# pjookim/srsran-ce-pytorch

Measured on AMD Instinct MI355X. Metric: slots/sec (273-PRB PUSCH, 4 Rx), higher is better.
Workload: dtype f32; 1 GPU; pusch273_4rx_filter; n_prb=273, n_sc=3276, n_sym=14, layers=1, rx_ports=4, smoothing=filter, interp=linear, slots_per_gpu=8192, global_slots=8192, rx_layout=[slot][port][sym][sc], parallelism=slot-shard x1, no collective

## Files before the change

srsran_ce_pytorch_amd/csrc/ce_denoise.hip:

```cpp
#include <hip/hip_runtime.h>
#include <stdint.h>
#include <string.h>

#include <type_traits>
#include <vector>

#include "ce_denoise.h"
#include "ce_stage.h"

typedef _Float16 half8 __attribute__((ext_vector_type(8)));
typedef _Float16 half4 __attribute__((ext_vector_type(4)));
typedef _Float16 half2v __attribute__((ext_vector_type(2)));
typedef float f32x4 __attribute__((ext_vector_type(4)));

struct ce_denoiser {
  int device = 0;
  half8* wfrag = nullptr;
  float* bias = nullptr;
};

#ifndef DN_ABLATE
#define DN_ABLATE 0
#endif

namespace {

#ifndef DN_MIN_WAVES
#define DN_MIN_WAVES 3
#endif
#ifndef DN_TWO_BODIES
#define DN_TWO_BODIES 0
#endif
#ifndef DN_L3_BUF
#define DN_L3_BUF 2
#endif
#ifndef DN_T_ROWS
#define DN_T_ROWS 32
#endif
constexpr int DN_T = DN_T_ROWS;
constexpr int DN_NB3 = DN_T / 16;
static_assert(DN_T % 16 == 0, "strip height");
constexpr int DN_NT = 256, DN_COLS = 16, DN_C = CE_DN_CHANNELS;
constexpr int X0_PIX = (DN_T + 6) * DN_COLS + 2;
constexpr int X1_PIX = (DN_T + 5) * DN_COLS + 2;
constexpr int X2_PIX = (DN_T + 2) * DN_COLS + 2;

__device__ __forceinline__ int tap_off(int tap) {
  const int ky = tap / 3, kx = tap - 3 * ky;
  return (ky - 1) * DN_COLS + (kx - 1);
}

constexpr int ROW_BYTES16 = DN_COLS * DN_C * 2;
constexpr int ROW_BYTES0 = DN_COLS * 4;

typedef _Float16 half2x __attribute__((ext_vector_type(2)));
__device__ __forceinline__ float2 masked(float2 v, bool ok) {
  const unsigned m = ok ? 0xFFFFFFFFu : 0u;
  return make_float2(__uint_as_float(__float_as_uint(v.x) & m), __uint_as_float(__float_as_uint(v.y) & m));
}
__device__ __forceinline__ half4 relu_h4(f32x4 acc, unsigned keep) {
  half2x lo = half2x{(_Float16)acc[0], (_Float16)acc[1]}, hi = half2x{(_Float16)acc[2], (_Float16)acc[3]};
  const half2x z = half2x{0, 0}, top = half2x{65504, 65504};
  lo = __builtin_elementwise_min(__builtin_elementwise_max(lo, z), top);
  hi = __builtin_elementwise_min(__builtin_elementwise_max(hi, z), top);
  unsigned ulo, uhi;
  __builtin_memcpy(&ulo, &lo, 4);
  __builtin_memcpy(&uhi, &hi, 4);
  ulo &= keep;
  uhi &= keep;
  __builtin_memcpy(&lo, &ulo, 4);
  __builtin_memcpy(&hi, &uhi, 4);
  return half4{lo[0], lo[1], hi[0], hi[1]};
}

__global__ __launch_bounds__(DN_NT, DN_MIN_WAVES) void ce_denoise_kernel(float2* __restrict__ ch, const half8* __restrict__ wfrag,
                                                            const float* __restrict__ bias, int n_sc, int L) {
  __shared__ __attribute__((aligned(16))) half2v x0[2][X0_PIX];
  __shared__ __attribute__((aligned(16))) _Float16 x1[X1_PIX * DN_C];
  __shared__ __attribute__((aligned(16))) _Float16 x2[X2_PIX * DN_C];
  const int tid = threadIdx.x, lane = tid & 63;
  const int wave = __builtin_amdgcn_readfirstlane(tid >> 6);
  const int n = lane & 15, g = lane >> 4;
  const int64_t plane = blockIdx.x;
  const int64_t item = plane / L;
  const int l = (int)(plane - item * L);
  float2* base = ch + item * (int64_t)n_sc * CE_DN_SYMBOLS * L + l;

  half8 w1 = wfrag[lane], w2[5], w3[9];
#pragma unroll
  for (int m = 0; m < 5; ++m) w2[m] = wfrag[(1 + m) * 64 + lane];
#pragma unroll
  for (int m = 0; m < 9; ++m) w3[m] = wfrag[(6 + m) * 64 + lane];
  f32x4 b1, b2, b3;
#pragma unroll
  for (int i = 0; i < 4; ++i) {
    b1[i] = bias[4 * g + i];
    b2[i] = bias[16 + 4 * g + i];
    b3[i] = g < 2 ? bias[32 + (i & 1)] : 0.f;
  }
  for (int i = tid; i < 2 * X0_PIX; i += DN_NT) (&x0[0][0])[i] = half2v{0, 0};
  for (int i = tid; i < X1_PIX * DN_C; i += DN_NT) x1[i] = 0;
  for (int i = tid; i < X2_PIX * DN_C; i += DN_NT) x2[i] = 0;

  const bool col_ok = n >= 1 && n <= CE_DN_SYMBOLS;
  const unsigned keep = col_ok ? 0xFFFFFFFFu : 0u;
  int rd0[4];
#pragma unroll
  for (int q = 0; q < 4; ++q) {
    const int tap = 4 * g + q;
    rd0[q] = (1 + (wave + 1) * DN_COLS + n + tap_off(tap < 9 ? tap : 4)) * 4;
  }
  constexpr int R2 = (DN_T + 2 + 3) / 4;
  const int a2 = wave * R2 < DN_T + 2 - R2 ? wave * R2 : DN_T + 2 - R2;
  int rdA, rdC, wr2;
  {
    const int pa = 1 + a2 * DN_COLS + n - 1 + (g >> 1), pc = 1 + (a2 + (g >> 1)) * DN_COLS + n + 1, pw = 1 + a2 * DN_COLS + n;
    rdA = pa * (DN_C * 2) + (((g & 1) ^ ((pa >> 2) & 1)) * 16);
    rdC = pc * (DN_C * 2) + (((g & 1) ^ ((pc >> 2) & 1)) * 16);
    wr2 = pw * (DN_C * 2) + ((((g >> 1) & 1) ^ ((pw >> 2) & 1)) * 16) + (g & 1) * 8;
  }
  const int wpix = 1 + wave * DN_COLS + n;
  const int wr = wpix * (DN_C * 2) + ((((g >> 1) & 1) ^ ((wpix >> 2) & 1)) * 16) + (g & 1) * 8;
  constexpr int ST_N = ((DN_T + 6) * DN_COLS + DN_NT - 1) / DN_NT;
  int st_off[ST_N], st_row[ST_N];
  bool st_ok[ST_N];
#pragma unroll
  for (int k = 0; k < ST_N; ++k) {
    const int i = tid + k * DN_NT, sym = (i & 15) - 1;
    st_row[k] = (i >> 4) - 3;
    st_ok[k] = i < (DN_T + 6) * DN_COLS && sym >= 0 && sym < CE_DN_SYMBOLS;
    st_off[k] = (st_row[k] * CE_DN_SYMBOLS + sym) * L;
  }
  int rd3[3];
#pragma unroll
  for (int dx = 0; dx < 3; ++dx) {
    const int pix = 1 + (4 * wave + 3 * (g >> 1)) * DN_COLS + n + dx - 1;
    rd3[dx] = pix * (DN_C * 2) + (((g & 1) ^ ((pix >> 2) & 1)) * 16);
  }
  const int h_row = 4 * wave + 2 * g;
  const int h_off = (h_row * CE_DN_SYMBOLS + (n - 1)) * L;
  const bool h_lane = g < 2 && col_ok;

  float2 st[ST_N];
  auto stage_load = [&](int r0) {
    const float2* sb = base + (int64_t)r0 * CE_DN_SYMBOLS * L;
#pragma unroll
    for (int k = 0; k < ST_N; ++k) {
      const bool ok = st_ok[k] && (unsigned)(r0 + st_row[k]) < (unsigned)n_sc;
      st[k] = masked((DN_ABLATE & 2) ? make_float2(0.f, 0.f) : sb[ok ? st_off[k] : 0], ok);
    }
  };
  auto stage_load_in = [&](int r0) {
    const float2* sb = base + (int64_t)r0 * CE_DN_SYMBOLS * L;
#pragma unroll
    for (int k = 0; k < ST_N; ++k) st[k] = masked((DN_ABLATE & 2) ? make_float2(0.f, 0.f) : sb[st_ok[k] ? st_off[k] : 0], st_ok[k]);
  };
  auto stage_store = [&](int buf) {
#pragma unroll
    for (int k = 0; k < ST_N; ++k) {
      const int i = tid + k * DN_NT;
      if (i < (DN_T + 6) * DN_COLS) x0[buf][1 + i] = half2v{(_Float16)st[k].x, (_Float16)st[k].y};
    }
  };
  stage_load(0);
  __syncthreads();
  stage_store(0);
  __syncthreads();
  const int n_strips = (n_sc + DN_T - 1) / DN_T;
  auto strip = [&](auto edge_tag, int s) __attribute__((always_inline)) {
    constexpr bool EDGE = decltype(edge_tag)::value;
    const int r0 = s * DN_T, buf = s & 1;
    float2* sb = base + (int64_t)r0 * CE_DN_SYMBOLS * L;
    if (s + 1 < n_strips) {
      if (!EDGE && r0 + 2 * DN_T + 3 <= n_sc) stage_load_in(r0 + DN_T); else stage_load(r0 + DN_T);
    }
    float2 hres[DN_NB3][2];
#pragma unroll
    for (int b = 0; b < DN_NB3; ++b)
#pragma unroll
      for (int e = 0; e < 2; ++e) {
        const bool ok = h_lane && (!EDGE || r0 + h_row + 16 * b + e < n_sc);
        hres[b][e] = masked((DN_ABLATE & 2) ? make_float2(0.f, 0.f) : sb[ok ? h_off + (16 * b + e) * CE_DN_SYMBOLS * L : 0], ok);
      }
    {
      const char* xin = reinterpret_cast<const char*>(&x0[buf][0]);
      char* xout = reinterpret_cast<char*>(x1);
      constexpr int NK1 = (DN_T + 4) / 4;
      auto finish1 = [&](f32x4 acc, int k) __attribute__((always_inline)) {
        const int row = r0 - 2 + wave + 4 * k;
        const unsigned rowkeep = (!EDGE || (row >= 0 && row < n_sc)) ? keep : 0u;
        *reinterpret_cast<half4*>(xout + wr + k * 4 * ROW_BYTES16) = relu_h4(acc, rowkeep);
      };
      f32x4 accp = b1;
      half2v px[2][4];
#pragma unroll
      for (int q = 0; q < 4; ++q) px[0][q] = *reinterpret_cast<const half2v*>(xin + rd0[q]);
#pragma unroll
      for (int k = 0; k < NK1; ++k) {
        if (k + 1 < NK1) {
#pragma unroll
          for (int q = 0; q < 4; ++q) px[(k + 1) & 1][q] = *reinterpret_cast<const half2v*>(xin + rd0[q] + (k + 1) * 4 * ROW_BYTES0);
        }
        asm volatile("" ::: "memory");
        half8 b;
#pragma unroll
        for (int q = 0; q < 4; ++q) {
          b[2 * q] = px[k & 1][q][0];
          b[2 * q + 1] = px[k & 1][q][1];
        }
        const f32x4 acc = __builtin_amdgcn_mfma_f32_16x16x32_f16(w1, b, b1, 0, 0, 0);
        if (k > 0) finish1(accp, k - 1);
        accp = acc;
      }
      finish1(accp, NK1 - 1);
    }
    __syncthreads();
    if (s + 1 < n_strips) stage_store(buf ^ 1);
    {
      const char* xin = reinterpret_cast<const char*>(x1);
      char* xout = reinterpret_cast<char*>(x2);
      half8 fa[R2 + 2], fc[R2 + 2];
      auto fetch = [&](int i) __attribute__((always_inline)) {
        fa[i] = *reinterpret_cast<const half8*>(xin + rdA + i * ROW_BYTES16);
        fc[i] = *reinterpret_cast<const half8*>(xin + rdC + i * ROW_BYTES16);
      };
      fetch(0);
      fetch(1);
      fetch(2);
      auto finish2 = [&](f32x4 acc, int j) __attribute__((always_inline)) {
        const int row = r0 - 1 + a2 + j;
        const unsigned rowkeep = (!EDGE || (row >= 0 && row < n_sc)) ? keep : 0u;
        *reinterpret_cast<half4*>(xout + wr2 + j * ROW_BYTES16) = relu_h4(acc, rowkeep);
      };
      f32x4 accp = b2;
#pragma unroll
      for (int j = 0; j < R2; ++j) {
        if (j + 3 < R2 + 2) fetch(j + 3);
        asm volatile("" ::: "memory");
        f32x4 acc = b2;
        acc = __builtin_amdgcn_mfma_f32_16x16x32_f16(w2[0], fa[j], acc, 0, 0, 0);
        acc = __builtin_amdgcn_mfma_f32_16x16x32_f16(w2[1], fa[j + 1], acc, 0, 0, 0);
        acc = __builtin_amdgcn_mfma_f32_16x16x32_f16(w2[2], fa[j + 2], acc, 0, 0, 0);
        acc = __builtin_amdgcn_mfma_f32_16x16x32_f16(w2[3], fc[j], acc, 0, 0, 0);
        acc = __builtin_amdgcn_mfma_f32_16x16x32_f16(w2[4], fc[j + 2], acc, 0, 0, 0);
        if (j > 0) finish2(accp, j - 1);
        accp = acc;
      }
      finish2(accp, R2 - 1);
    }
    __syncthreads();
    {
      const char* xin = reinterpret_cast<const char*>(x2);
      auto finish3 = [&](f32x4 acc, int b) __attribute__((always_inline)) {
#pragma unroll
        for (int e = 0; e < 2; ++e)
          if ((!(DN_ABLATE & 1) || acc[0] == 123.456f) && h_lane && (!EDGE || r0 + h_row + 16 * b + e < n_sc))
            sb[h_off + (16 * b + e) * CE_DN_SYMBOLS * L] = make_float2(hres[b][e].x + acc[2 * e], hres[b][e].y + acc[2 * e + 1]);
      };
      f32x4 accp = b3;
      half8 fr[DN_L3_BUF][9];
#pragma unroll
      for (int j = 0; j < 9; ++j) fr[0][j] = *reinterpret_cast<const half8*>(xin + rd3[j % 3] + (j / 3) * ROW_BYTES16);
#pragma unroll
      for (int b = 0; b < DN_NB3; ++b) {
        if (DN_L3_BUF == 2 && b + 1 < DN_NB3) {
#pragma unroll
          for (int j = 0; j < 9; ++j) fr[(b + 1) & 1][j] = *reinterpret_cast<const half8*>(xin + rd3[j % 3] + (16 * (b + 1) + j / 3) * ROW_BYTES16);
        }
        if (DN_L3_BUF == 1 && b > 0) {
#pragma unroll
          for (int j = 0; j < 9; ++j) fr[0][j] = *reinterpret_cast<const half8*>(xin + rd3[j % 3] + (16 * b + j / 3) * ROW_BYTES16);
        }
        asm volatile("" ::: "memory");
        f32x4 acc = b3;
#pragma unroll
        for (int j = 0; j < 9; ++j) acc = __builtin_amdgcn_mfma_f32_16x16x32_f16(w3[j], fr[b & (DN_L3_BUF - 1)][j], acc, 0, 0, 0);
        if (b > 0) finish3(accp, b - 1);
        accp = acc;
      }
      finish3(accp, DN_NB3 - 1);
    }
  };
#pragma unroll 1
  for (int s = 0; s < n_strips; ++s) {
    const int r0 = s * DN_T;
    if (DN_TWO_BODIES && r0 >= 3 && r0 + DN_T + 3 <= n_sc) strip(std::false_type{}, s);
    else strip(std::true_type{}, s);
  }
}

_Float16 to_h(float v) { return (_Float16)v; }

}

extern "C" int ce_denoiser_create(int32_t device, const float* w1, const float* b1, const float* w2, const float* b2,
                                  const float* w3, const float* b3, ce_denoiser** out) {
  if (!w1 || !b1 || !w2 || !b2 || !w3 || !b3 || !out) return ce_fail(CE_ERR_INVALID, "null argument");
  std::vector<_Float16> frag(15 * 64 * 8, to_h(0.f));
  auto at = [&](int f, int lane, int j) -> _Float16& { return frag[((size_t)f * 64 + lane) * 8 + j]; };
  for (int lane = 0; lane < 64; ++lane) {
    const int co = lane & 15, g = lane >> 4;
    for (int j = 0; j < 8; ++j) {
      const int k = 8 * g + j, tap = k >> 1, ci = k & 1;
      if (tap < 9) at(0, lane, j) = to_h(w1[(co * 2 + ci) * 9 + tap]);
    }
    for (int j = 0; j < 8; ++j) {
      const int ci = 8 * (g & 1) + j, up = g >> 1;
      for (int ky = 0; ky < 3; ++ky) at(1 + ky, lane, j) = to_h(w2[(co * 16 + ci) * 9 + ky * 3 + up]);
      at(4, lane, j) = to_h(w2[(co * 16 + ci) * 9 + up * 3 + 2]);
      if (!up) at(5, lane, j) = to_h(w2[(co * 16 + ci) * 9 + 2 * 3 + 2]);
    }
    if (co < 8)
      for (int m = 0; m < 9; ++m)
        for (int j = 0; j < 8; ++j) {
          const int r = co >> 1, c3 = co & 1, ri = m / 3 + 3 * (g >> 1), dx = m % 3, ci = 8 * (g & 1) + j, ky = ri - r;
          if (ky >= 0 && ky <= 2) at(6 + m, lane, j) = to_h(w3[(c3 * 16 + ci) * 9 + ky * 3 + dx]);
        }
  }
  float bias[48] = {0};
  for (int i = 0; i < 16; ++i) { bias[i] = b1[i]; bias[16 + i] = b2[i]; }
  bias[32] = b3[0];
  bias[33] = b3[1];
  ce_denoiser* d = new ce_denoiser;
  d->device = device;
  CeDeviceScope scope(device);
  hipError_t e = ce_upload(scope.err, &d->wfrag, frag.data(), frag.size() * sizeof(_Float16));
  e = ce_upload(e, &d->bias, bias, sizeof(bias));
  if (e != hipSuccess) {
    ce_denoiser_destroy(d);
    return ce_fail(CE_ERR_HIP, "denoiser upload: %s", hipGetErrorString(e));
  }
  *out = d;
  return CE_OK;
}

extern "C" void ce_denoiser_destroy(ce_denoiser* d) {
  if (!d) return;
  if (d->wfrag) (void)hipFree(d->wfrag);
  if (d->bias) (void)hipFree(d->bias);
  delete d;
}

extern "C" int ce_denoise_batch(const ce_denoiser* d, void* ch_est, int64_t n_items, int32_t n_sc, int32_t n_sym,
                                int32_t n_layers, void* stream) {
  if (!d || (!ch_est && n_items > 0)) return ce_fail(CE_ERR_INVALID, "null argument");
  if (n_sym != CE_DN_SYMBOLS) return ce_fail(CE_ERR_UNSUPPORTED, "the denoiser is built for 14-symbol grids (got %d)", n_sym);
  if (n_items < 0 || n_sc < 1 || n_layers < 1 || n_layers > CE_MAX_LAYERS) return ce_fail(CE_ERR_INVALID, "bad shape");
  const int64_t planes = n_items * n_layers;
  if (planes == 0) return CE_OK;
  if (planes > 0x7FFFFFFFll) return ce_fail(CE_ERR_UNSUPPORTED, "%lld planes in one launch", (long long)planes);
  CeDeviceScope scope(d->device);
  if (scope.err != hipSuccess) return ce_device_fail(d->device, scope.err);
  hipLaunchKernelGGL(ce_denoise_kernel, dim3((unsigned)planes), dim3(DN_NT), 0, (hipStream_t)stream,
                     reinterpret_cast<float2*>(ch_est), d->wfrag, d->bias, n_sc, n_layers);
  return ce_launch_status("denoise");
}
```

Before: 3.614 million slots/s.

## Recast final conv as 2-MFMA row-pair GEMM with DPP tap reduction, single-buffer x0

Reformulates the third conv layer so each output row pair is produced by two MFMAs over row-shifted input fragments. The horizontal taps become separate output columns that are then summed across lanes with DPP shifts, instead of nine MFMAs per 16-row block. Layer-3 weight fragments shrink from 9 to 2 per lane, and the input staging buffer x0 drops from double to single buffering. Together with raising the launch-bounds minimum from 3 to 4, this targets lower register and LDS pressure and higher occupancy. The risks are a more serialized staging path, since the store now waits on the sync after layer 1, and extra cross-lane DPP work in the epilogue.

```diff
diff --git a/srsran_ce_pytorch_amd/csrc/ce_denoise.hip b/srsran_ce_pytorch_amd/csrc/ce_denoise.hip
--- a/srsran_ce_pytorch_amd/csrc/ce_denoise.hip
+++ b/srsran_ce_pytorch_amd/csrc/ce_denoise.hip
@@ -26,19 +26,20 @@
 namespace {
 
 #ifndef DN_MIN_WAVES
-#define DN_MIN_WAVES 3
+#define DN_MIN_WAVES 4
 #endif
 #ifndef DN_TWO_BODIES
 #define DN_TWO_BODIES 0
 #endif
-#ifndef DN_L3_BUF
-#define DN_L3_BUF 2
+#ifndef DN_W_RESIDENT
+#define DN_W_RESIDENT 1
 #endif
 #ifndef DN_T_ROWS
 #define DN_T_ROWS 32
 #endif
 constexpr int DN_T = DN_T_ROWS;
-constexpr int DN_NB3 = DN_T / 16;
+constexpr int DN_RW3 = DN_T / 4;
+constexpr int DN_NP3 = DN_RW3 / 2;
 static_assert(DN_T % 16 == 0, "strip height");
 constexpr int DN_NT = 256, DN_COLS = 16, DN_C = CE_DN_CHANNELS;
 constexpr int X0_PIX = (DN_T + 6) * DN_COLS + 2;
@@ -75,7 +76,7 @@
 
 __global__ __launch_bounds__(DN_NT, DN_MIN_WAVES) void ce_denoise_kernel(float2* __restrict__ ch, const half8* __restrict__ wfrag,
                                                             const float* __restrict__ bias, int n_sc, int L) {
-  __shared__ __attribute__((aligned(16))) half2v x0[2][X0_PIX];
+  __shared__ __attribute__((aligned(16))) half2v x0[X0_PIX];
   __shared__ __attribute__((aligned(16))) _Float16 x1[X1_PIX * DN_C];
   __shared__ __attribute__((aligned(16))) _Float16 x2[X2_PIX * DN_C];
   const int tid = threadIdx.x, lane = tid & 63;
@@ -86,19 +87,24 @@
   const int l = (int)(plane - item * L);
   float2* base = ch + item * (int64_t)n_sc * CE_DN_SYMBOLS * L + l;
 
-  half8 w1 = wfrag[lane], w2[5], w3[9];
-#pragma unroll
-  for (int m = 0; m < 5; ++m) w2[m] = wfrag[(1 + m) * 64 + lane];
-#pragma unroll
-  for (int m = 0; m < 9; ++m) w3[m] = wfrag[(6 + m) * 64 + lane];
-  f32x4 b1, b2, b3;
-#pragma unroll
-  for (int i = 0; i < 4; ++i) {
-    b1[i] = bias[4 * g + i];
-    b2[i] = bias[16 + 4 * g + i];
-    b3[i] = g < 2 ? bias[32 + (i & 1)] : 0.f;
-  }
-  for (int i = tid; i < 2 * X0_PIX; i += DN_NT) (&x0[0][0])[i] = half2v{0, 0};
+  half8 w1, w2[5], w3[2];
+  f32x4 b1, b2;
+  float b3c;
+  auto load_weights = [&](const half8* wf, const float* bs) __attribute__((always_inline)) {
+    w1 = wf[lane];
+#pragma unroll
+    for (int m = 0; m < 5; ++m) w2[m] = wf[(1 + m) * 64 + lane];
+#pragma unroll
+    for (int m = 0; m < 2; ++m) w3[m] = wf[(6 + m) * 64 + lane];
+#pragma unroll
+    for (int i = 0; i < 4; ++i) {
+      b1[i] = bs[4 * g + i];
+      b2[i] = bs[16 + 4 * g + i];
+    }
+    b3c = bs[32 + (g & 1)];
+  };
+  load_weights(wfrag, bias);
+  for (int i = tid; i < X0_PIX; i += DN_NT) x0[i] = half2v{0, 0};
   for (int i = tid; i < X1_PIX * DN_C; i += DN_NT) x1[i] = 0;
   for (int i = tid; i < X2_PIX * DN_C; i += DN_NT) x2[i] = 0;
 
@@ -131,35 +137,36 @@
     st_ok[k] = i < (DN_T + 6) * DN_COLS && sym >= 0 && sym < CE_DN_SYMBOLS;
     st_off[k] = (st_row[k] * CE_DN_SYMBOLS + sym) * L;
   }
-  int rd3[3];
-#pragma unroll
-  for (int dx = 0; dx < 3; ++dx) {
-    const int pix = 1 + (4 * wave + 3 * (g >> 1)) * DN_COLS + n + dx - 1;
-    rd3[dx] = pix * (DN_C * 2) + (((g & 1) ^ ((pix >> 2) & 1)) * 16);
-  }
-  const int h_row = 4 * wave + 2 * g;
-  const int h_off = (h_row * CE_DN_SYMBOLS + (n - 1)) * L;
-  const bool h_lane = g < 2 && col_ok;
+  int rd3;
+  {
+    const int pix = 1 + (DN_RW3 * wave + (g >> 1)) * DN_COLS + n;
+    rd3 = pix * (DN_C * 2) + (((g & 1) ^ ((pix >> 2) & 1)) * 16);
+  }
+  const int h_row = DN_RW3 * wave + (g >> 1);
+  const int h_off = (h_row * CE_DN_SYMBOLS + (n - 1)) * L * 2 + (g & 1);
+  const bool h_lane = col_ok;
 
   float2 st[ST_N];
+  constexpr int DN_NO_STRIP = 1 << 30;
   auto stage_load = [&](int r0) {
-    const float2* sb = base + (int64_t)r0 * CE_DN_SYMBOLS * L;
+    const float2* sb = base + (int64_t)(r0 == DN_NO_STRIP ? 0 : r0) * CE_DN_SYMBOLS * L;
 #pragma unroll
     for (int k = 0; k < ST_N; ++k) {
       const bool ok = st_ok[k] && (unsigned)(r0 + st_row[k]) < (unsigned)n_sc;
-      st[k] = masked((DN_ABLATE & 2) ? make_float2(0.f, 0.f) : sb[ok ? st_off[k] : 0], ok);
+      st[k] = (DN_ABLATE & 2) ? make_float2(0.f, 0.f) : sb[ok ? st_off[k] : 0];
     }
   };
   auto stage_load_in = [&](int r0) {
     const float2* sb = base + (int64_t)r0 * CE_DN_SYMBOLS * L;
 #pragma unroll
-    for (int k = 0; k < ST_N; ++k) st[k] = masked((DN_ABLATE & 2) ? make_float2(0.f, 0.f) : sb[st_ok[k] ? st_off[k] : 0], st_ok[k]);
-  };
-  auto stage_store = [&](int buf) {
+    for (int k = 0; k < ST_N; ++k) st[k] = (DN_ABLATE & 2) ? make_float2(0.f, 0.f) : sb[st_ok[k] ? st_off[k] : 0];
+  };
+  auto stage_store = [&](int r0) {
 #pragma unroll
     for (int k = 0; k < ST_N; ++k) {
       const int i = tid + k * DN_NT;
-      if (i < (DN_T + 6) * DN_COLS) x0[buf][1 + i] = half2v{(_Float16)st[k].x, (_Float16)st[k].y};
+      const float2 v = masked(st[k], st_ok[k] && (unsigned)(r0 + st_row[k]) < (unsigned)n_sc);
+      if (i < (DN_T + 6) * DN_COLS) x0[1 + i] = half2v{(_Float16)v.x, (_Float16)v.y};
     }
   };
   stage_load(0);
@@ -169,21 +176,24 @@
   const int n_strips = (n_sc + DN_T - 1) / DN_T;
   auto strip = [&](auto edge_tag, int s) __attribute__((always_inline)) {
     constexpr bool EDGE = decltype(edge_tag)::value;
-    const int r0 = s * DN_T, buf = s & 1;
+    const int r0 = s * DN_T;
     float2* sb = base + (int64_t)r0 * CE_DN_SYMBOLS * L;
-    if (s + 1 < n_strips) {
-      if (!EDGE && r0 + 2 * DN_T + 3 <= n_sc) stage_load_in(r0 + DN_T); else stage_load(r0 + DN_T);
-    }
-    float2 hres[DN_NB3][2];
-#pragma unroll
-    for (int b = 0; b < DN_NB3; ++b)
-#pragma unroll
-      for (int e = 0; e < 2; ++e) {
-        const bool ok = h_lane && (!EDGE || r0 + h_row + 16 * b + e < n_sc);
-        hres[b][e] = masked((DN_ABLATE & 2) ? make_float2(0.f, 0.f) : sb[ok ? h_off + (16 * b + e) * CE_DN_SYMBOLS * L : 0], ok);
-      }
+    if (!DN_W_RESIDENT) {
+      int w_zero = 0;
+      asm volatile("" : "+s"(w_zero));
+      load_weights(wfrag + w_zero, bias + w_zero);
+    }
+    if (!EDGE && r0 + 2 * DN_T + 3 <= n_sc) stage_load_in(r0 + DN_T); else stage_load(s + 1 < n_strips ? r0 + DN_T : DN_NO_STRIP);
+    float* sbf = reinterpret_cast<float*>(sb);
+    float hres[DN_NP3];
+#pragma unroll
+    for (int p = 0; p < DN_NP3; ++p) {
+      const bool ok = h_lane && (!EDGE || r0 + h_row + 2 * p < n_sc);
+      const float v = (DN_ABLATE & 2) ? 0.f : sbf[ok ? h_off + 2 * p * CE_DN_SYMBOLS * L * 2 : 0];
+      hres[p] = __uint_as_float(__float_as_uint(v) & (ok ? 0xFFFFFFFFu : 0u));
+    }
     {
-      const char* xin = reinterpret_cast<const char*>(&x0[buf][0]);
+      const char* xin = reinterpret_cast<const char*>(&x0[0]);
       char* xout = reinterpret_cast<char*>(x1);
       constexpr int NK1 = (DN_T + 4) / 4;
       auto finish1 = [&](f32x4 acc, int k) __attribute__((always_inline)) {
@@ -215,7 +225,7 @@
       finish1(accp, NK1 - 1);
     }
     __syncthreads();
-    if (s + 1 < n_strips) stage_store(buf ^ 1);
+    if (s + 1 < n_strips) stage_store(r0 + DN_T);
     {
       const char* xin = reinterpret_cast<const char*>(x1);
       char* xout = reinterpret_cast<char*>(x2);
@@ -251,34 +261,26 @@
     __syncthreads();
     {
       const char* xin = reinterpret_cast<const char*>(x2);
-      auto finish3 = [&](f32x4 acc, int b) __attribute__((always_inline)) {
-#pragma unroll
-        for (int e = 0; e < 2; ++e)
-          if ((!(DN_ABLATE & 1) || acc[0] == 123.456f) && h_lane && (!EDGE || r0 + h_row + 16 * b + e < n_sc))
-            sb[h_off + (16 * b + e) * CE_DN_SYMBOLS * L] = make_float2(hres[b][e].x + acc[2 * e], hres[b][e].y + acc[2 * e + 1]);
+      const f32x4 b3 = f32x4{0.f, b3c, 0.f, 0.f};
+      auto finish3 = [&](f32x4 acc, int p) __attribute__((always_inline)) {
+        const float left = __int_as_float(__builtin_amdgcn_update_dpp(0, __float_as_int(acc[0]), 0x111, 0xf, 0xf, true));
+        const float right = __int_as_float(__builtin_amdgcn_update_dpp(0, __float_as_int(acc[2]), 0x101, 0xf, 0xf, true));
+        if ((!(DN_ABLATE & 1) || acc[0] == 123.456f) && h_lane && (!EDGE || r0 + h_row + 2 * p < n_sc))
+          sbf[h_off + 2 * p * CE_DN_SYMBOLS * L * 2] = hres[p] + ((acc[1] + left) + right);
       };
+      half8 fr[DN_NP3 + 1];
+#pragma unroll
+      for (int q = 0; q < DN_NP3 + 1; ++q) fr[q] = *reinterpret_cast<const half8*>(xin + rd3 + 2 * q * ROW_BYTES16);
+      __builtin_amdgcn_sched_barrier(0);
       f32x4 accp = b3;
-      half8 fr[DN_L3_BUF][9];
-#pragma unroll
-      for (int j = 0; j < 9; ++j) fr[0][j] = *reinterpret_cast<const half8*>(xin + rd3[j % 3] + (j / 3) * ROW_BYTES16);
-#pragma unroll
-      for (int b = 0; b < DN_NB3; ++b) {
-        if (DN_L3_BUF == 2 && b + 1 < DN_NB3) {
-#pragma unroll
-          for (int j = 0; j < 9; ++j) fr[(b + 1) & 1][j] = *reinterpret_cast<const half8*>(xin + rd3[j % 3] + (16 * (b + 1) + j / 3) * ROW_BYTES16);
-        }
-        if (DN_L3_BUF == 1 && b > 0) {
-#pragma unroll
-          for (int j = 0; j < 9; ++j) fr[0][j] = *reinterpret_cast<const half8*>(xin + rd3[j % 3] + (16 * b + j / 3) * ROW_BYTES16);
-        }
-        asm volatile("" ::: "memory");
-        f32x4 acc = b3;
-#pragma unroll
-        for (int j = 0; j < 9; ++j) acc = __builtin_amdgcn_mfma_f32_16x16x32_f16(w3[j], fr[b & (DN_L3_BUF - 1)][j], acc, 0, 0, 0);
-        if (b > 0) finish3(accp, b - 1);
+#pragma unroll
+      for (int p = 0; p < DN_NP3; ++p) {
+        f32x4 acc = __builtin_amdgcn_mfma_f32_16x16x32_f16(w3[0], fr[p], b3, 0, 0, 0);
+        acc = __builtin_amdgcn_mfma_f32_16x16x32_f16(w3[1], fr[p + 1], acc, 0, 0, 0);
+        if (p > 0) finish3(accp, p - 1);
         accp = acc;
       }
-      finish3(accp, DN_NB3 - 1);
+      finish3(accp, DN_NP3 - 1);
     }
   };
 #pragma unroll 1
@@ -296,7 +298,7 @@
 extern "C" int ce_denoiser_create(int32_t device, const float* w1, const float* b1, const float* w2, const float* b2,
                                   const float* w3, const float* b3, ce_denoiser** out) {
   if (!w1 || !b1 || !w2 || !b2 || !w3 || !b3 || !out) return ce_fail(CE_ERR_INVALID, "null argument");
-  std::vector<_Float16> frag(15 * 64 * 8, to_h(0.f));
+  std::vector<_Float16> frag(8 * 64 * 8, to_h(0.f));
   auto at = [&](int f, int lane, int j) -> _Float16& { return frag[((size_t)f * 64 + lane) * 8 + j]; };
   for (int lane = 0; lane < 64; ++lane) {
     const int co = lane & 15, g = lane >> 4;
@@ -310,11 +312,11 @@
       at(4, lane, j) = to_h(w2[(co * 16 + ci) * 9 + up * 3 + 2]);
       if (!up) at(5, lane, j) = to_h(w2[(co * 16 + ci) * 9 + 2 * 3 + 2]);
     }
-    if (co < 8)
-      for (int m = 0; m < 9; ++m)
+    if ((co & 3) < 3)
+      for (int f = 0; f < 2; ++f)
         for (int j = 0; j < 8; ++j) {
-          const int r = co >> 1, c3 = co & 1, ri = m / 3 + 3 * (g >> 1), dx = m % 3, ci = 8 * (g & 1) + j, ky = ri - r;
-          if (ky >= 0 && ky <= 2) at(6 + m, lane, j) = to_h(w3[(c3 * 16 + ci) * 9 + ky * 3 + dx]);
+          const int e = co >> 3, c3 = (co >> 2) & 1, dx = co & 3, ci = 8 * (g & 1) + j, ky = 2 * f + (g >> 1) - e;
+          if (ky >= 0 && ky <= 2) at(6 + f, lane, j) = to_h(w3[(c3 * 16 + ci) * 9 + ky * 3 + dx]);
         }
   }
   float bias[48] = {0};
```

Result: no change. 3.615 million slots/s (median of 3 runs) (+0.0%).
